# SCZwangxiao/video-ReTaKe

Measured on NVIDIA B200. Metric: 2048-frame DPSelect+PivotKV frames/s, higher is better.
Workload: dtype bf16

## Files before the change

video-retake_b200/csrc/pivot_misc.cu:

```cuda
#include <climits>

#include <stdlib.h>

#include "rtk_common.cuh"

namespace rtk {

struct RopeParams {
    int heads, L, D, n_pos, forward;
    long long stride_h, stride_l, out_stride_h, out_stride_l;
    int heads2;
    const __nv_bfloat16* x2;
    __nv_bfloat16* out2;
    long long stride_h2, stride_l2, out_stride_h2, out_stride_l2;
    int bound[6];
    float inv_scale2;
};

static bool mrope_bounds(int n_pos, const int32_t* sec, int64_t D, int bound[6]) {
    int acc = 0;
    for (int i = 0; i < 6; ++i) {
        acc += n_pos == 3 ? sec[i % 3] : 0;
        bound[i] = acc;
    }
    return n_pos != 3 || acc == D;
}

__device__ __forceinline__ int rope_pos_row(const RopeParams& p, int c) {
    if (p.n_pos == 1) return 0;
    int i = 0;
    while (i < 5 && c >= p.bound[i]) ++i;
    return i % 3;
}

__global__ void __launch_bounds__(256)
pivot_rope_table_kernel(const long long* __restrict__ pos, const float* __restrict__ inv_freq, RopeParams p, float scaling,
                        __nv_bfloat16* __restrict__ cos_t, __nv_bfloat16* __restrict__ sin_t) {
    pdl_enter();
    const int half = p.D >> 1;
    const long long total = (long long)p.L * p.D;
    for (long long i = (long long)blockIdx.x * blockDim.x + threadIdx.x; i < total; i += (long long)gridDim.x * blockDim.x) {
        const int c = (int)(i % p.D);
        const int l = (int)(i / p.D);
        const long long pv = pos[(size_t)rope_pos_row(p, c) * p.L + l];
        const float ang = inv_freq[c < half ? c : c - half] * (float)pv;
        cos_t[i] = __float2bfloat16_rn(cosf(ang) * scaling);
        sin_t[i] = __float2bfloat16_rn(sinf(ang) * scaling);
    }
}

__device__ __forceinline__ void rope_rotate_pair(float xa, float xb, float cosa, float sina, float cosb, float sinb, int forward,
                                                 float inv_scale2, __nv_bfloat16& oa, __nv_bfloat16& ob) {
    const float ta = round_bf16(xa * cosa), ra = round_bf16(-xb * sina);
    const float tb = round_bf16(xb * cosb), rb = round_bf16(xa * sinb);
    float ya, yb;
    if (forward) {
        ya = ta + ra;
        yb = tb + rb;
    } else {
        ya = round_bf16(ta - ra) * inv_scale2;
        yb = round_bf16(tb - rb) * inv_scale2;
    }
    oa = __float2bfloat16_rn(ya);
    ob = __float2bfloat16_rn(yb);
}

__device__ __forceinline__ void rope_table_entry(const RopeParams& p, const float* __restrict__ inv_freq, const long long* pv,
                                                 int c, float scaling, float& co, float& si) {
    const int half = p.D >> 1;
    const float ang = inv_freq[c < half ? c : c - half] * (float)pv[rope_pos_row(p, c)];
    co = __bfloat162float(__float2bfloat16_rn(cosf(ang) * scaling));
    si = __bfloat162float(__float2bfloat16_rn(sinf(ang) * scaling));
}

#ifndef RTK_UNROPE_TOK
#define RTK_UNROPE_TOK 2
#endif
constexpr int kUnropeTok = RTK_UNROPE_TOK;

__device__ __forceinline__ uint32_t sub_bf16x2_rn(uint32_t a, uint32_t b) {
    uint32_t d;
    asm("sub.rn.bf16x2 %0, %1, %2;" : "=r"(d) : "r"(a), "r"(b));
    return d;
}
__device__ __forceinline__ uint32_t add_bf16x2_rn(uint32_t a, uint32_t b) {
    uint32_t d;
    asm("add.rn.bf16x2 %0, %1, %2;" : "=r"(d) : "r"(a), "r"(b));
    return d;
}
__device__ __forceinline__ void unrotate_bf16x2(uint32_t xa, uint32_t xb, uint32_t cs, uint32_t sn, bool scale, float inv_scale2,
                                                uint32_t& oa, uint32_t& ob) {
    const uint32_t ta = mul_bf16x2_rn(xa, cs), ra = mul_bf16x2_rn(xb ^ 0x80008000u, sn);
    const uint32_t tb = mul_bf16x2_rn(xb, cs), rb = mul_bf16x2_rn(xa, sn);
    oa = sub_bf16x2_rn(ta, ra);
    ob = sub_bf16x2_rn(tb, rb);
    if (scale) {
        oa = scale_bf16x2_rn(oa, inv_scale2);
        ob = scale_bf16x2_rn(ob, inv_scale2);
    }
}

__device__ __forceinline__ void unrope_qk_body(const __nv_bfloat16* __restrict__ x, const long long* __restrict__ pos,
                                               const float* __restrict__ inv_freq, float scaling,
                                               __nv_bfloat16* __restrict__ out, const RopeParams& p) {
    __shared__ __align__(16) __nv_bfloat16 s_cos[kUnropeTok][128], s_sin[kUnropeTok][128];
    const int half = p.D >> 1;
    const int vec_per_row = half >> 3;
    const int ntask = (p.heads + p.heads2) * vec_per_row;
    const int tid = threadIdx.x;
    const bool scale = p.inv_scale2 != 1.0f;
    const int v0 = tid % vec_per_row, h0 = tid / vec_per_row;
    const bool second0 = h0 >= p.heads;
    const long long src_h0 = second0 ? (long long)(h0 - p.heads) * p.stride_h2 : (long long)h0 * p.stride_h;
    const long long src_l0 = second0 ? p.stride_l2 : p.stride_l;
    const __nv_bfloat16* src0 = (second0 ? p.x2 : x) + src_h0 + v0 * 8;
    for (int l0 = blockIdx.x * kUnropeTok; l0 < p.L; l0 += gridDim.x * kUnropeTok) {
        const int nl = min(kUnropeTok, p.L - l0);
        uint4 lo4[kUnropeTok], hi4[kUnropeTok];
        if (tid < ntask) {
#pragma unroll
            for (int t = 0; t < kUnropeTok; ++t) {
                if (t < nl) {
                    lo4[t] = *reinterpret_cast<const uint4*>(src0 + (l0 + t) * src_l0);
                    hi4[t] = *reinterpret_cast<const uint4*>(src0 + (l0 + t) * src_l0 + half);
                }
            }
        }
        for (int e = tid; e < nl * half; e += blockDim.x) {
            const int t = e / half, c = e - t * half;
            long long pv[3] = {0, 0, 0};
            for (int r = 0; r < p.n_pos; ++r) pv[r] = pos[(size_t)r * p.L + l0 + t];
            float co, si;
            rope_table_entry(p, inv_freq, pv, c, scaling, co, si);
            s_cos[t][c] = __float2bfloat16_rn(co);
            s_sin[t][c] = __float2bfloat16_rn(si);
        }
        __syncthreads();
#pragma unroll
        for (int t = 0; t < kUnropeTok; ++t) {
            if (t >= nl) break;
            const int l = l0 + t;
            for (int task = tid; task < ntask; task += blockDim.x) {
                const int v = task % vec_per_row, h = task / vec_per_row;
                const int c0 = v * 8;
                const bool second = h >= p.heads;
                const __nv_bfloat16* src = second ? p.x2 + (h - p.heads) * p.stride_h2 + l * p.stride_l2 : x + h * p.stride_h + l * p.stride_l;
                __nv_bfloat16* dst = second ? p.out2 + (h - p.heads) * p.out_stride_h2 + l * p.out_stride_l2
                                            : out + h * p.out_stride_h + l * p.out_stride_l;
                uint4 a4 = lo4[t], b4 = hi4[t];
                if (task != tid) {
                    a4 = *reinterpret_cast<const uint4*>(src + c0);
                    b4 = *reinterpret_cast<const uint4*>(src + c0 + half);
                }
                const uint4 cs = *reinterpret_cast<const uint4*>(&s_cos[t][c0]);
                const uint4 sn = *reinterpret_cast<const uint4*>(&s_sin[t][c0]);
                uint4 ol4, oh4;
                unrotate_bf16x2(a4.x, b4.x, cs.x, sn.x, scale, p.inv_scale2, ol4.x, oh4.x);
                unrotate_bf16x2(a4.y, b4.y, cs.y, sn.y, scale, p.inv_scale2, ol4.y, oh4.y);
                unrotate_bf16x2(a4.z, b4.z, cs.z, sn.z, scale, p.inv_scale2, ol4.z, oh4.z);
                unrotate_bf16x2(a4.w, b4.w, cs.w, sn.w, scale, p.inv_scale2, ol4.w, oh4.w);
                *reinterpret_cast<uint4*>(dst + c0) = ol4;
                *reinterpret_cast<uint4*>(dst + c0 + half) = oh4;
            }
        }
        __syncthreads();
    }
}

struct BatchLayers {
    const __nv_bfloat16* q[kMaxBatchLayers];
    const __nv_bfloat16* k[kMaxBatchLayers];
    const __nv_bfloat16* k_in[kMaxBatchLayers];
    const __nv_bfloat16* v[kMaxBatchLayers];
    __nv_bfloat16* qu[kMaxBatchLayers];
    __nv_bfloat16* ku[kMaxBatchLayers];
    const long long* pos[kMaxBatchLayers];
    const uint8_t* keymask[kMaxBatchLayers];
    __nv_bfloat16* k_out[kMaxBatchLayers];
    __nv_bfloat16* v_out[kMaxBatchLayers];
    long long* pos_out[kMaxBatchLayers];
    int32_t* keep_idx[kMaxBatchLayers];
    const __nv_bfloat16* head_scores[kMaxBatchLayers];
    long long q_stride_h[kMaxBatchLayers], q_stride_l[kMaxBatchLayers];
    long long kin_stride_h[kMaxBatchLayers], kin_stride_l[kMaxBatchLayers];
    long long k_stride_h[kMaxBatchLayers], k_stride_l[kMaxBatchLayers];
    long long v_stride_h[kMaxBatchLayers], v_stride_l[kMaxBatchLayers];
    long long out_stride_h[kMaxBatchLayers], pos_out_stride[kMaxBatchLayers];
};

__global__ void __launch_bounds__(256)
pivot_unrope_qk_batch_kernel(const __grid_constant__ BatchLayers t, const float* __restrict__ inv_freq, float scaling, RopeParams p) {
    pdl_enter();
    const int layer = blockIdx.y;
    p.stride_h = t.q_stride_h[layer]; p.stride_l = t.q_stride_l[layer];
    p.x2 = t.k_in[layer]; p.out2 = t.ku[layer];
    p.stride_h2 = t.kin_stride_h[layer]; p.stride_l2 = t.kin_stride_l[layer];
    unrope_qk_body(t.q[layer], t.pos[layer], inv_freq, scaling, t.qu[layer], p);
}

__global__ void __launch_bounds__(256)
pivot_rope_kernel(const __nv_bfloat16* __restrict__ x, const __nv_bfloat16* __restrict__ cos_t,
                  const __nv_bfloat16* __restrict__ sin_t, __nv_bfloat16* __restrict__ out, RopeParams p) {
    pdl_enter();
    const int half = p.D >> 1;
    const int vec_per_row = half >> 3;
    const long long total = (long long)(p.heads + p.heads2) * p.L * vec_per_row;
    for (long long i = (long long)blockIdx.x * blockDim.x + threadIdx.x; i < total; i += (long long)gridDim.x * blockDim.x) {
        const int v = (int)(i % vec_per_row);
        const long long hl = i / vec_per_row;
        const int l = (int)(hl % p.L);
        const int h = (int)(hl / p.L);
        const int c0 = v * 8;
        const bool second = h >= p.heads;
        const __nv_bfloat16* src = second ? p.x2 + (h - p.heads) * p.stride_h2 + l * p.stride_l2 : x + h * p.stride_h + l * p.stride_l;
        __nv_bfloat16* dst = second ? p.out2 + (h - p.heads) * p.out_stride_h2 + l * p.out_stride_l2
                                    : out + h * p.out_stride_h + l * p.out_stride_l;
        uint4 lo4 = *reinterpret_cast<const uint4*>(src + c0);
        uint4 hi4 = *reinterpret_cast<const uint4*>(src + c0 + half);
        const __nv_bfloat16* xl = reinterpret_cast<const __nv_bfloat16*>(&lo4);
        const __nv_bfloat16* xh = reinterpret_cast<const __nv_bfloat16*>(&hi4);
        uint4 ol4, oh4;
        __nv_bfloat16* ol = reinterpret_cast<__nv_bfloat16*>(&ol4);
        __nv_bfloat16* oh = reinterpret_cast<__nv_bfloat16*>(&oh4);
        const int rowa0 = rope_pos_row(p, c0), rowa1 = rope_pos_row(p, c0 + 7);
        const int rowb0 = rope_pos_row(p, c0 + half), rowb1 = rope_pos_row(p, c0 + half + 7);
        uint4 ca4, sa4, cb4, sb4;
        __nv_bfloat16* cav = reinterpret_cast<__nv_bfloat16*>(&ca4);
        __nv_bfloat16* sav = reinterpret_cast<__nv_bfloat16*>(&sa4);
        __nv_bfloat16* cbv = reinterpret_cast<__nv_bfloat16*>(&cb4);
        __nv_bfloat16* sbv = reinterpret_cast<__nv_bfloat16*>(&sb4);
        if (rowa0 == rowa1 && rowb0 == rowb1) {
            const size_t ia = ((size_t)rowa0 * p.L + l) * p.D + c0, ib = ((size_t)rowb0 * p.L + l) * p.D + c0 + half;
            ca4 = __ldg(reinterpret_cast<const uint4*>(cos_t + ia));
            sa4 = __ldg(reinterpret_cast<const uint4*>(sin_t + ia));
            cb4 = __ldg(reinterpret_cast<const uint4*>(cos_t + ib));
            sb4 = __ldg(reinterpret_cast<const uint4*>(sin_t + ib));
        } else {
#pragma unroll
            for (int e = 0; e < 8; ++e) {
                const int ca = c0 + e, cb = c0 + e + half;
                const size_t ia = ((size_t)rope_pos_row(p, ca) * p.L + l) * p.D + ca;
                const size_t ib = ((size_t)rope_pos_row(p, cb) * p.L + l) * p.D + cb;
                cav[e] = cos_t[ia]; sav[e] = sin_t[ia]; cbv[e] = cos_t[ib]; sbv[e] = sin_t[ib];
            }
        }
#pragma unroll
        for (int e = 0; e < 8; ++e)
            rope_rotate_pair(__bfloat162float(xl[e]), __bfloat162float(xh[e]), __bfloat162float(cav[e]), __bfloat162float(sav[e]),
                             __bfloat162float(cbv[e]), __bfloat162float(sbv[e]), p.forward, p.inv_scale2, ol[e], oh[e]);
        *reinterpret_cast<uint4*>(dst + c0) = ol4;
        *reinterpret_cast<uint4*>(dst + c0 + half) = oh4;
    }
}

bool key_elision_enabled();

struct KeyElide {
    const uint8_t* keymask[kMaxBatchLayers];
    int32_t* slot[kMaxBatchLayers];
    const __nv_bfloat16* k[kMaxBatchLayers];
    long long k_stride_h[kMaxBatchLayers], k_stride_l[kMaxBatchLayers];
    __nv_bfloat16* kc[kMaxBatchLayers];
    int32_t* n_keys;
    int L, KVH, D;
};

__global__ void __launch_bounds__(1024)
pivot_keymask_scan_kernel(const __grid_constant__ KeyElide e) {
    pdl_enter();
    __shared__ int wsum[32];
    const int layer = blockIdx.x, tid = threadIdx.x, lane = tid & 31, warp = tid >> 5;
    const uint8_t* __restrict__ m = e.keymask[layer];
    int32_t* __restrict__ slot = e.slot[layer];
    const int per = (e.L + 1023) / 1024;
    const int beg = min(tid * per, e.L), end = min(beg + per, e.L);
    int cnt = 0;
    for (int i = beg; i < end; ++i) cnt += !(m && m[i]);
    int inc = cnt;
#pragma unroll
    for (int o = 1; o < 32; o <<= 1) {
        const int n = __shfl_up_sync(0xffffffffu, inc, o);
        if (lane >= o) inc += n;
    }
    if (lane == 31) wsum[warp] = inc;
    __syncthreads();
    if (warp == 0) {
        const int w = wsum[lane];
        int winc = w;
#pragma unroll
        for (int o = 1; o < 32; o <<= 1) {
            const int n = __shfl_up_sync(0xffffffffu, winc, o);
            if (lane >= o) winc += n;
        }
        wsum[lane] = winc - w;
        if (lane == 31) e.n_keys[layer] = winc;
    }
    __syncthreads();
    int base = wsum[warp] + inc - cnt;
    for (int i = beg; i < end; ++i) slot[i] = (m && m[i]) ? -1 : base++;
}

__global__ void __launch_bounds__(256)
pivot_keys_compact_kernel(const __grid_constant__ KeyElide e) {
    pdl_enter();
    const int layer = blockIdx.y;
    const int vpr = e.D >> 3;
    const long long total = (long long)e.L * e.KVH * vpr;
    const int32_t* __restrict__ slot = e.slot[layer];
    for (long long i = (long long)blockIdx.x * blockDim.x + threadIdx.x; i < total; i += (long long)gridDim.x * blockDim.x) {
        const int v = (int)(i % vpr);
        const long long lh = i / vpr;
        const int h = (int)(lh % e.KVH);
        const int l = (int)(lh / e.KVH);
        const int sl = slot[l];
        if (sl < 0) continue;
        const uint4 w = __ldg(reinterpret_cast<const uint4*>(e.k[layer] + h * e.k_stride_h[layer] + l * e.k_stride_l[layer] + v * 8));
        *reinterpret_cast<uint4*>(e.kc[layer] + ((size_t)sl * e.KVH + h) * e.D + v * 8) = w;
    }
}

static int key_elide_prepare(KeyElide& ke, int n, ScoreBatch& sb, cudaStream_t st) {
    RTK_LAUNCH_PDL(pivot_keymask_scan_kernel, (unsigned)n, 1024, 0, st, ke);
    const long long total = (long long)ke.L * ke.KVH * (ke.D >> 3);
    long long gx = (total + 255) / 256;
    if (gx > 148 * 8) gx = 148 * 8;
    RTK_LAUNCH_PDL(pivot_keys_compact_kernel, dim3((unsigned)gx, (unsigned)n), 256, 0, st, ke);
    for (int i = 0; i < n; ++i) {
        sb.kc[i] = ke.kc[i];
        sb.slot[i] = ke.slot[i];
    }
    sb.n_keys = ke.n_keys;
    return 0;
}

static size_t key_elide_bytes(int64_t KVH, int64_t L, int64_t D) {
    return (((size_t)KVH * L * D * 2 + 255) & ~(size_t)255) + (((size_t)L * 4 + 255) & ~(size_t)255);
}

constexpr int kSelThreads = 1024;

__device__ void block_select_top(const uint32_t* keys, int L, int keep, int32_t* out_idx, int* sh ,
                                 int low_bit ) {
    const int tid = threadIdx.x, lane = tid & 31, warp = tid >> 5;
    const int per = (L + kSelThreads - 1) / kSelThreads;
    const int beg = min(tid * per, L), end = min(beg + per, L);
    uint32_t prefix = 0;
    for (int bit = 31; bit >= low_bit; --bit) {
        const uint32_t cand = prefix | (1u << bit);
        int cnt = 0;
        for (int i = beg; i < end; ++i) cnt += (keys[i] >= cand);
        cnt = __reduce_add_sync(0xffffffffu, cnt);
        int* buf = sh + 40 + 32 * (bit & 1);
        if (lane == 0) buf[warp] = cnt;
        __syncthreads();
        const int total = __reduce_add_sync(0xffffffffu, buf[lane]);
        if (total >= keep) prefix = cand;
    }
    __syncthreads();
    if (low_bit > 0 && (!(prefix & 0x80000000u) || (prefix >> low_bit) == (0xffffffffu >> low_bit)))
        prefix |= (1u << low_bit) - 1u;
    int gt = 0, eq = 0;
    for (int i = beg; i < end; ++i) { gt += (keys[i] > prefix); eq += (keys[i] == prefix); }
    auto block_excl_scan = [&](int v, int& total) {
        int inc = v;
#pragma unroll
        for (int o = 1; o < 32; o <<= 1) {
            const int n = __shfl_up_sync(0xffffffffu, inc, o);
            if (lane >= o) inc += n;
        }
        __syncthreads();
        if (lane == 31) sh[1 + warp] = inc;
        __syncthreads();
        if (warp == 0) {
            int w = sh[1 + lane], winc = w;
#pragma unroll
            for (int o = 1; o < 32; o <<= 1) {
                const int n = __shfl_up_sync(0xffffffffu, winc, o);
                if (lane >= o) winc += n;
            }
            sh[1 + lane] = winc - w;
            if (lane == 31) sh[33] = winc;
        }
        __syncthreads();
        total = sh[33];
        return sh[1 + warp] + inc - v;
    };
    int gt_total, eq_total;
    const int gt_before = block_excl_scan(gt, gt_total);
    const int eq_before = block_excl_scan(eq, eq_total);
    const int need = keep - gt_total;
    const int eq_taken_before = min(eq_before, need);
    int slot = gt_before + eq_taken_before;
    int eq_seen = eq_before;
    for (int i = beg; i < end; ++i) {
        const uint32_t k = keys[i];
        bool take = k > prefix;
        if (k == prefix) { take = eq_seen < need; ++eq_seen; }
        if (take) out_idx[slot++] = i;
    }
}

__device__ __forceinline__ void pivot_select_body(const __nv_bfloat16* __restrict__ head_scores, int KVH, int L,
                                                  const uint8_t* __restrict__ keymask, int keep, int32_t* __restrict__ keep_idx,
                                                  __nv_bfloat16* __restrict__ score_out, const long long* __restrict__ tpos,
                                                  long long* __restrict__ tmin_out) {
    extern __shared__ __align__(128) uint8_t smem[];
    uint32_t* keys = reinterpret_cast<uint32_t*>(smem);
    int* sh = reinterpret_cast<int*>(smem + (size_t)L * 4);
    const float rcp = 1.0f / (float)KVH;
    for (int i = threadIdx.x; i < L; i += blockDim.x) {
        float v[4] = {0.f, 0.f, 0.f, 0.f};
        for (int j = 0; j < KVH; ++j) v[j & 3] += __bfloat162float(head_scores[(size_t)j * L + i]);
        const __nv_bfloat16 s = __float2bfloat16_rn((((v[0] + v[1]) + v[2]) + v[3]) * rcp);
        if (score_out) score_out[i] = s;
        const float f = (keymask && keymask[i]) ? 1.0f : __bfloat162float(s);
        keys[i] = f32_to_ordered(f);
    }
// ... 302 lines not shown
    if (grid > 148 * 16) grid = 148 * 16;
    RTK_LAUNCH_PDL(pivot_rope_kernel, (unsigned)grid, 256, 0, st, (const __nv_bfloat16*)x, (const __nv_bfloat16*)cos, (const __nv_bfloat16*)sin, (__nv_bfloat16*)out, p);
    return 0;
}

extern "C" int rtk_pivot_rope(const void* x, int64_t heads, int64_t L, int64_t D, int64_t stride_h, int64_t stride_l,
                              const void* cos, const void* sin, int n_pos, const int32_t* mrope_section_host,
                              float inv_scale2, int forward, void* out, int64_t out_stride_h, int64_t out_stride_l,
                              void* stream) {
    RTK_NVTX("rtk_pivot_rope");
    if (!x || !cos || !sin || !out || heads < 1 || L < 1 || D < 16) return RTK_E_BADARG;
    if (D % 16 != 0 || (n_pos != 1 && n_pos != 3)) return RTK_E_UNSUPPORTED;
    if (n_pos == 3 && !mrope_section_host) return RTK_E_BADARG;
    if ((((uintptr_t)x | (uintptr_t)out) & 15u) != 0) return RTK_E_ALIGN;
    if ((stride_h | stride_l | out_stride_h | out_stride_l) % 8 != 0) return RTK_E_ALIGN;
    RopeParams p;
    p.heads = (int)heads; p.L = (int)L; p.D = (int)D; p.n_pos = n_pos; p.forward = forward;
    p.stride_h = stride_h; p.stride_l = stride_l; p.out_stride_h = out_stride_h; p.out_stride_l = out_stride_l;
    p.inv_scale2 = inv_scale2;
    p.heads2 = 0; p.x2 = nullptr; p.out2 = nullptr;
    p.stride_h2 = p.stride_l2 = p.out_stride_h2 = p.out_stride_l2 = 0;
    if (!mrope_bounds(n_pos, mrope_section_host, D, p.bound)) return RTK_E_UNSUPPORTED;
    return rope_launch(x, cos, sin, out, p, (cudaStream_t)stream);
}

extern "C" int rtk_pivot_select(const void* head_scores, int64_t KVH, int64_t L, const uint8_t* keymask, int64_t keep,
                                int32_t* keep_idx, void* score_out, void* stream) {
    RTK_NVTX("rtk_pivot_select");
    if (!head_scores || !keep_idx || KVH < 1 || L < 1 || keep < 1 || keep > L) return RTK_E_BADARG;
    if (L > 16384) return RTK_E_UNSUPPORTED;
    const size_t smem = (size_t)L * 4 + 112 * 4;
    cudaError_t e = cudaFuncSetAttribute(pivot_select_kernel, cudaFuncAttributeMaxDynamicSharedMemorySize, (int)smem);
    if (e != cudaSuccess) return (int)e;
    RTK_LAUNCH_PDL(pivot_select_kernel, 1, kSelThreads, smem, (cudaStream_t)stream, (const __nv_bfloat16*)head_scores, (int)KVH,
                   (int)L, keymask, (int)keep, keep_idx, (__nv_bfloat16*)score_out);
    return 0;
}

extern "C" int rtk_pivot_compact(const void* k, const void* v, int64_t KVH, int64_t L, int64_t D, int64_t stride_h,
                                 int64_t stride_l, const int32_t* keep_idx, int64_t keep, void* k_out, void* v_out,
                                 int64_t out_stride_h, const int64_t* pos, int n_pos, int64_t* pos_out, int reforge,
                                 void* stream) {
    RTK_NVTX("rtk_pivot_compact");
    if ((!k && !v) || !keep_idx || (k && !k_out) || (v && !v_out) || KVH < 1 || L < 1 || D < 8 || keep < 1 || keep > L)
        return RTK_E_BADARG;
    if (pos && (!pos_out || n_pos < 1)) return RTK_E_BADARG;
    if (D % 8 != 0) return RTK_E_UNSUPPORTED;
    if ((((uintptr_t)k | (uintptr_t)v | (uintptr_t)k_out | (uintptr_t)v_out) & 15u) != 0) return RTK_E_ALIGN;
    if ((stride_h | stride_l | out_stride_h) % 8 != 0) return RTK_E_ALIGN;
    CompactParams p;
    p.KVH = (int)KVH; p.L = (int)L; p.D = (int)D; p.keep = (int)keep; p.n_pos = n_pos; p.reforge = reforge;
    p.stride_h = stride_h; p.stride_l = stride_l; p.out_stride_h = out_stride_h;
    p.v_stride_h = stride_h; p.v_stride_l = stride_l;
    p.pos_out_stride = keep;
    p.ratio = (float)((double)keep / (double)L);
    const long long total = KVH * keep * (D / 8);
    long long grid = (total + 255) / 256;
    if (grid > 148 * 8) grid = 148 * 8;
    RTK_LAUNCH_PDL(pivot_compact_kernel, (unsigned)(grid + 1), 256, 0, (cudaStream_t)stream,  (const __nv_bfloat16*)k, (const __nv_bfloat16*)v, keep_idx, (__nv_bfloat16*)k_out, (__nv_bfloat16*)v_out, (const long long*)pos, (long long*)pos_out, p);
    return 0;
}

extern "C" int rtk_pivot_rope_tables(const int64_t* pos, int n_pos, int64_t L, int64_t D, const float* inv_freq,
                                     const int32_t* mrope_section_host, float attention_scaling, void* cos_out,
                                     void* sin_out, void* stream) {
    RTK_NVTX("rtk_pivot_rope_tables");
    if (!pos || !inv_freq || !cos_out || !sin_out || L < 1 || D < 2) return RTK_E_BADARG;
    if (D % 2 != 0 || (n_pos != 1 && n_pos != 3)) return RTK_E_UNSUPPORTED;
    if (n_pos == 3 && !mrope_section_host) return RTK_E_BADARG;
    RopeParams p;
    p.heads = 1; p.L = (int)L; p.D = (int)D; p.n_pos = n_pos; p.forward = 0;
    p.stride_h = p.stride_l = p.out_stride_h = p.out_stride_l = 0;
    p.heads2 = 0; p.x2 = nullptr; p.out2 = nullptr;
    p.stride_h2 = p.stride_l2 = p.out_stride_h2 = p.out_stride_l2 = 0;
    p.inv_scale2 = 1.0f;
    if (!mrope_bounds(n_pos, mrope_section_host, D, p.bound)) return RTK_E_UNSUPPORTED;
    long long grid = (L * D + 255) / 256;
    if (grid > 148 * 8) grid = 148 * 8;
    RTK_LAUNCH_PDL(pivot_rope_table_kernel, (unsigned)grid, 256, 0, (cudaStream_t)stream,  (const long long*)pos, inv_freq, p, attention_scaling, (__nv_bfloat16*)cos_out, (__nv_bfloat16*)sin_out);
    return 0;
}

static size_t align256(size_t x) { return (x + 255) & ~(size_t)255; }

extern "C" size_t rtk_pivot_update_batch_workspace_bytes(int64_t H, int64_t KVH, int64_t L, int64_t D, int64_t n_layers) {
    if (H < 1 || KVH < 1 || L < 1 || D < 1 || n_layers < 1) return 0;
    const size_t n = (size_t)(n_layers < kMaxBatchLayers ? n_layers : kMaxBatchLayers);
    return align256(rtk_pivot_score_workspace_bytes(H * (int64_t)n, L)) +
           n * (align256((size_t)H * L * D * 2) + align256((size_t)KVH * L * D * 2)) + align256(n * sizeof(long long)) + 256 +
           n * key_elide_bytes(KVH, L, D) + 256;
}

extern "C" size_t rtk_pivot_update_workspace_bytes(int64_t H, int64_t KVH, int64_t L, int64_t D) {
    return rtk_pivot_update_batch_workspace_bytes(H, KVH, L, D, 1);
}

#ifndef RTK_UNROT_TOKEN_MAJOR
#define RTK_UNROT_TOKEN_MAJOR 1
#endif

static int pivot_update_group(const rtk_pivot_update_args* a, int n, char* ws, cudaStream_t st) {
    const rtk_pivot_update_args& a0 = a[0];
    const int64_t H = a0.H, KVH = a0.KVH, L = a0.L, D = a0.D;
    const bool reforge = a0.reforge != 0;
    const int64_t uq_sh = RTK_UNROT_TOKEN_MAJOR ? D : L * D, uq_sl = RTK_UNROT_TOKEN_MAJOR ? H * D : D;
    const int64_t uk_sh = RTK_UNROT_TOKEN_MAJOR ? D : L * D, uk_sl = RTK_UNROT_TOKEN_MAJOR ? KVH * D : D;
    void* score_ws = ws;                ws += align256(rtk_pivot_score_workspace_bytes(H * n, L));
    char* qu0 = ws;                     ws += (size_t)n * align256((size_t)H * L * D * 2);
    char* ku0 = ws;                     ws += (size_t)n * align256((size_t)KVH * L * D * 2);
    long long* tmin = (long long*)ws;   ws += align256((size_t)n * sizeof(long long)) + 256;
    char* kc0 = ws;                     ws += (size_t)n * align256((size_t)KVH * L * D * 2);
    char* slot0 = ws;                   ws += (size_t)n * align256((size_t)L * 4);
    int32_t* nkeys_ws = (int32_t*)ws;

    BatchLayers t = {};
    ScoreBatch sb = {};
    sb.n = n; sb.H = H; sb.KVH = KVH; sb.L = L; sb.D = D;
    for (int i = 0; i < kMaxBatchLayers; ++i) {
        const rtk_pivot_update_args& x = a[i < n ? i : 0];
        char* qu = qu0 + (size_t)(i < n ? i : 0) * align256((size_t)H * L * D * 2);
        char* ku = ku0 + (size_t)(i < n ? i : 0) * align256((size_t)KVH * L * D * 2);
        t.q[i] = (const __nv_bfloat16*)x.q;       t.q_stride_h[i] = x.q_stride_h;     t.q_stride_l[i] = x.q_stride_l;
        t.k_in[i] = (const __nv_bfloat16*)x.k;    t.kin_stride_h[i] = x.k_stride_h;   t.kin_stride_l[i] = x.k_stride_l;
        t.qu[i] = (__nv_bfloat16*)qu;             t.ku[i] = (__nv_bfloat16*)ku;
        t.k[i] = reforge ? (const __nv_bfloat16*)ku : (const __nv_bfloat16*)x.k;
        t.k_stride_h[i] = reforge ? uk_sh : x.k_stride_h;
        t.k_stride_l[i] = reforge ? uk_sl : x.k_stride_l;
        t.v[i] = (const __nv_bfloat16*)x.v;       t.v_stride_h[i] = x.v_stride_h;     t.v_stride_l[i] = x.v_stride_l;
        t.pos[i] = (const long long*)x.pos;       t.keymask[i] = x.keymask;
        t.k_out[i] = (__nv_bfloat16*)x.k_out;     t.v_out[i] = (__nv_bfloat16*)x.v_out;
        t.out_stride_h[i] = x.out_stride_h;
        t.pos_out[i] = (long long*)x.pos_out;     t.pos_out_stride[i] = x.pos_out_stride > 0 ? x.pos_out_stride : x.keep;
        t.keep_idx[i] = x.keep_idx;               t.head_scores[i] = (const __nv_bfloat16*)x.head_scores;
        if (i < n) {
            sb.q[i] = reforge ? (const void*)qu : x.q;
            sb.k[i] = reforge ? (const void*)ku : x.k;
            sb.q_stride_h[i] = reforge ? uq_sh : x.q_stride_h;   sb.q_stride_l[i] = reforge ? uq_sl : x.q_stride_l;
            sb.k_stride_h[i] = reforge ? uk_sh : x.k_stride_h;   sb.k_stride_l[i] = reforge ? uk_sl : x.k_stride_l;
            sb.head_scores[i] = x.head_scores;
        }
    }
    RopeParams rp = {};
    rp.heads = (int)H; rp.L = (int)L; rp.D = (int)D; rp.n_pos = a0.n_pos; rp.forward = 0;
    rp.out_stride_h = uq_sh; rp.out_stride_l = uq_sl;
    rp.heads2 = (int)KVH; rp.out_stride_h2 = uk_sh; rp.out_stride_l2 = uk_sl;
    rp.inv_scale2 = a0.inv_scale2;
    mrope_bounds(a0.n_pos, a0.mrope_section, D, rp.bound);
    const bool xchg = a0.xchg_world > 1;
    const int64_t score_rows = a0.score_rows > 0 ? a0.score_rows : KVH;
    if (reforge && !a0.skip_score) {
        if (a0.inv_freq) {
            RTK_LAUNCH_PDL(pivot_unrope_qk_batch_kernel, dim3((unsigned)((L + kUnropeTok - 1) / kUnropeTok), (unsigned)n), 256, 0, st, t, a0.inv_freq,
                           a0.attention_scaling, rp);
        } else {
            rp.stride_h = a0.q_stride_h; rp.stride_l = a0.q_stride_l;
            rp.x2 = t.k_in[0]; rp.out2 = t.ku[0]; rp.stride_h2 = a0.k_stride_h; rp.stride_l2 = a0.k_stride_l;
            const int rc = rope_launch(a0.q, a0.cos, a0.sin, t.qu[0], rp, st);
            if (rc) return rc;
        }
    }
    if (!a0.skip_score) {
        bool any_mask = false;
        for (int i = 0; i < n; ++i) any_mask = any_mask || a[i].keymask != nullptr;
        if (any_mask && key_elision_enabled()) {
            KeyElide ke = {};
            ke.L = (int)L; ke.KVH = (int)KVH; ke.D = (int)D; ke.n_keys = nkeys_ws;
            for (int i = 0; i < kMaxBatchLayers; ++i) {
                const int j = i < n ? i : 0;
                ke.keymask[i] = a[j].keymask;
                ke.slot[i] = (int32_t*)(slot0 + (size_t)j * align256((size_t)L * 4));
                ke.k[i] = t.k[j]; ke.k_stride_h[i] = t.k_stride_h[j]; ke.k_stride_l[i] = t.k_stride_l[j];
                ke.kc[i] = (__nv_bfloat16*)(kc0 + (size_t)j * align256((size_t)KVH * L * D * 2));
            }
            int rc = key_elide_prepare(ke, n, sb, st);
            if (rc) return rc;
        }
        if (a0.ev_score_begin) cudaEventRecord((cudaEvent_t)a0.ev_score_begin, st);
        int rc = pivot_score_batch(sb, score_ws, rtk_pivot_score_workspace_bytes(H * n, L), st);
        if (rc) return rc;
        if (a0.ev_score_end) cudaEventRecord((cudaEvent_t)a0.ev_score_end, st);
    }
    if (a0.skip_select) {
        if (xchg) {
            XchgPutBatch xp = {};
            xp.n = (long long)KVH * L; xp.world = a0.xchg_world; xp.rank = a0.xchg_rank;
            for (int i = 0; i < n; ++i) {
                xp.src[i] = (const __nv_bfloat16*)a[i].head_scores;
                for (int r = 0; r < a0.xchg_world; ++r)
                    xp.dst[i][r] = (__nv_bfloat16*)a[i].xchg_scores[r] + (size_t)a0.xchg_rank * KVH * L;
            }
            RTK_LAUNCH_PDL(pivot_xchg_put_batch_kernel, (unsigned)n, 1024, 0, st, xp);
            XchgFlags xf = {};
            xf.world = a0.xchg_world; xf.rank = a0.xchg_rank; xf.epoch = a0.xchg_epoch;
            for (int r = 0; r < a0.xchg_world; ++r) xf.flags[r] = a0.xchg_flags[r];
            RTK_LAUNCH_PDL(pivot_xchg_flag_kernel, 1, 32, 0, st, xf);
        }
        return 0;
    }
    {
        const size_t smem = (size_t)L * 4 + 112 * 4;
        cudaError_t e = cudaFuncSetAttribute(pivot_select_batch_kernel, cudaFuncAttributeMaxDynamicSharedMemorySize, (int)smem);
        if (e != cudaSuccess) return (int)e;
        RTK_LAUNCH_PDL(pivot_select_batch_kernel, (unsigned)n, kSelThreads, smem, st, t, (int)score_rows, (int)L, (int)a0.keep,
                       reforge ? 1 : 0, tmin, (const uint32_t*)(xchg ? a0.xchg_flags[a0.xchg_rank] : nullptr),
                       xchg ? a0.xchg_world : 0, a0.xchg_epoch, xchg_timeout_ns());
    }
    {
        CompactParams p = {};
        p.KVH = (int)KVH; p.L = (int)L; p.D = (int)D; p.keep = (int)a0.keep; p.n_pos = a0.pos ? a0.n_pos : 0; p.reforge = a0.reforge;
        p.ratio = (float)((double)a0.keep / (double)L);
        RopeParams rq = {};
        rq.D = (int)D; rq.n_pos = a0.n_pos; rq.L = (int)a0.keep;
        for (int i = 0; i < 6; ++i) rq.bound[i] = rp.bound[i];
        RTK_LAUNCH_PDL(pivot_compact_rope_batch_kernel, dim3((unsigned)a0.keep, (unsigned)n), 128, 0, st, t, (const long long*)tmin,
                       a0.inv_freq, a0.attention_scaling, p, rq, (reforge && a0.inv_freq) ? 1 : 0);
    }
    return 0;
}

static int update_check(const rtk_pivot_update_args* layers, int64_t n, const void* workspace, size_t workspace_bytes) {
    if (!layers || n < 1 || !workspace) return RTK_E_BADARG;
    const rtk_pivot_update_args& a0 = layers[0];
    const bool scores = !a0.skip_score, selects = !a0.skip_select, xchg = a0.xchg_world > 1;
    if (!scores && !selects) return RTK_E_BADARG;
    if (a0.H < 1 || a0.KVH < 1 || a0.L < 1 || (selects && (a0.keep < 1 || a0.keep > a0.L))) return RTK_E_BADARG;
    if (a0.L > 16384 || a0.D % 16 != 0 || a0.D > 256) return RTK_E_UNSUPPORTED;
    if (scores && ((a0.D != 64 && a0.D != 128) || a0.H % a0.KVH != 0 || a0.H > 256)) return RTK_E_UNSUPPORTED;
    if (xchg) {
        if (n > kMaxBatchLayers) return RTK_E_UNSUPPORTED;
        if (a0.xchg_world > 8 || a0.xchg_rank < 0 || a0.xchg_rank >= a0.xchg_world || (scores && selects)) return RTK_E_BADARG;
    }
    if (a0.reforge && !a0.inv_freq && n > 1) return RTK_E_UNSUPPORTED;
    int bound[6];
    if (a0.reforge && (scores || a0.inv_freq) && !mrope_bounds(a0.n_pos, a0.mrope_section, a0.D, bound)) return RTK_E_UNSUPPORTED;
    if (((uintptr_t)workspace & 255u) != 0) return RTK_E_ALIGN;
    if (workspace_bytes < rtk_pivot_update_batch_workspace_bytes(a0.H, a0.KVH, a0.L, a0.D, n)) return RTK_E_WORKSPACE;
    for (int64_t i = 0; i < n; ++i) {
        const rtk_pivot_update_args& x = layers[i];
        if (!x.q || !x.k || !x.v || !x.k_out || !x.v_out || !x.keep_idx || !x.head_scores) return RTK_E_BADARG;
        if (x.H != a0.H || x.KVH != a0.KVH || x.L != a0.L || x.D != a0.D || x.keep != a0.keep || x.reforge != a0.reforge ||
            x.n_pos != a0.n_pos || x.inv_freq != a0.inv_freq || x.attention_scaling != a0.attention_scaling ||
            x.inv_scale2 != a0.inv_scale2 || x.skip_select != a0.skip_select || x.skip_score != a0.skip_score ||
            x.score_rows != a0.score_rows || x.xchg_world != a0.xchg_world || x.xchg_rank != a0.xchg_rank ||
            x.xchg_epoch != a0.xchg_epoch || (x.pos == nullptr) != (a0.pos == nullptr))
            return RTK_E_UNSUPPORTED;
        for (int j = 0; j < 3; ++j)
            if (x.mrope_section[j] != a0.mrope_section[j]) return RTK_E_UNSUPPORTED;
        if (x.reforge && (!x.pos || !x.pos_out || (!x.inv_freq && (!x.cos || !x.sin)))) return RTK_E_BADARG;
        if (xchg) {
            for (int r = 0; r < a0.xchg_world; ++r)
                if (!x.xchg_scores[r] || !a0.xchg_flags[r]) return RTK_E_BADARG;
            const char* own = (const char*)x.xchg_scores[a0.xchg_rank];
            if (a0.skip_score && (const char*)x.head_scores != own) return RTK_E_BADARG;
            if (a0.skip_select && (const char*)x.head_scores != own + (size_t)a0.xchg_rank * a0.KVH * a0.L * 2) return RTK_E_BADARG;
        }
        if (x.pos && (selects || x.reforge) && (!x.pos_out || x.n_pos < 1 || x.n_pos > 3)) return RTK_E_BADARG;
        uintptr_t ptrs = 0;
        int64_t strides = 0;
        if (scores) {
            ptrs |= (uintptr_t)x.q;
            strides |= x.q_stride_h | x.q_stride_l;
        }
        if (scores || !x.reforge) {
            ptrs |= (uintptr_t)x.k;
            strides |= x.k_stride_h | x.k_stride_l;
        }
        if (selects) {
            ptrs |= (uintptr_t)x.v | (uintptr_t)x.k_out | (uintptr_t)x.v_out;
            strides |= x.v_stride_h | x.v_stride_l | x.out_stride_h;
        }
        if ((ptrs & 15u) != 0 || strides % 8 != 0) return RTK_E_ALIGN;
    }
    return 0;
}

extern "C" int rtk_pivot_update(const rtk_pivot_update_args* a, void* stream) {
    RTK_NVTX("rtk_pivot_update");
    if (!a) return RTK_E_BADARG;
    const int rc = update_check(a, 1, a->workspace, a->workspace_bytes);
    if (rc) return rc;
    return pivot_update_group(a, 1, (char*)a->workspace, (cudaStream_t)stream);
}

extern "C" int rtk_pivot_update_batch(const rtk_pivot_update_args* layers, int64_t n_layers, void* workspace,
                                      size_t workspace_bytes, void* stream) {
    RTK_NVTX("rtk_pivot_update_batch");
    int rc = update_check(layers, n_layers, workspace, workspace_bytes);
    if (rc) return rc;
    for (int64_t i = 0; i < n_layers; i += kMaxBatchLayers) {
        const int n = (int)((n_layers - i) < kMaxBatchLayers ? (n_layers - i) : kMaxBatchLayers);
        rc = pivot_update_group(layers + i, n, (char*)workspace, (cudaStream_t)stream);
        if (rc) return rc;
    }
    return 0;
}

extern "C" int rtk_kv_block_copy(int n_jobs, const void* const* src, void* const* dst, const int64_t* heads, const int64_t* rows,
                                 const int64_t* src_stride_h, const int64_t* src_stride_l, const int64_t* dst_stride_h,
                                 const int64_t* dst_stride_l, int64_t D, void* stream) {
    RTK_NVTX("rtk_kv_block_copy");
    if (n_jobs < 1 || n_jobs > 4 || !src || !dst || !heads || !rows || D < 8) return RTK_E_BADARG;
    if (D % 8 != 0) return RTK_E_UNSUPPORTED;
    CopyJobs j;
    j.n = n_jobs;
    j.D = (int)D;
    long long acc = 0;
    for (int k = 0; k < n_jobs; ++k) {
        if (!src[k] || !dst[k] || heads[k] < 1 || rows[k] < 0) return RTK_E_BADARG;
        if ((((uintptr_t)src[k] | (uintptr_t)dst[k]) & 15u) != 0) return RTK_E_ALIGN;
        if ((src_stride_h[k] | src_stride_l[k] | dst_stride_h[k] | dst_stride_l[k]) % 8 != 0) return RTK_E_ALIGN;
        j.src[k] = (const __nv_bfloat16*)src[k];
        j.dst[k] = (__nv_bfloat16*)dst[k];
        j.heads[k] = (int)heads[k];
        j.rows[k] = (int)rows[k];
        j.src_stride_h[k] = src_stride_h[k]; j.src_stride_l[k] = src_stride_l[k];
        j.dst_stride_h[k] = dst_stride_h[k]; j.dst_stride_l[k] = dst_stride_l[k];
        acc += heads[k] * rows[k] * (D / 8);
// ... 10 lines not shown
```

Measured before the change: 3613.

## Precompute deduplicated unrope cos/sin tables and fuse key compaction into unrope

Adds a table kernel that reduces each position row to its min/max. When the values span fewer than L entries, it builds cos/sin tables indexed by position value, so each distinct position is computed once instead of once per token per block. The per-token unrope kernel then reads cos/sin from these global tables instead of computing them in shared memory with a __syncthreads. When key elision is active, the unrope kernel also writes the unroped keys straight into the compacted key buffer, which replaces the separate keys-compact kernel. This costs more workspace and one extra launch, and tokens whose 8-element vector straddles mRoPE sections fall back to gathering scalar table entries.

```diff
diff --git a/video-retake_b200/csrc/pivot_misc.cu b/video-retake_b200/csrc/pivot_misc.cu
--- a/video-retake_b200/csrc/pivot_misc.cu
+++ b/video-retake_b200/csrc/pivot_misc.cu
@@ -77,6 +77,7 @@
 #define RTK_UNROPE_TOK 2
 #endif
 constexpr int kUnropeTok = RTK_UNROPE_TOK;
+constexpr int kUnropeTableCtas = 16;
 
 __device__ __forceinline__ uint32_t sub_bf16x2_rn(uint32_t a, uint32_t b) {
     uint32_t d;
@@ -100,72 +101,22 @@
     }
 }
 
-__device__ __forceinline__ void unrope_qk_body(const __nv_bfloat16* __restrict__ x, const long long* __restrict__ pos,
-                                               const float* __restrict__ inv_freq, float scaling,
-                                               __nv_bfloat16* __restrict__ out, const RopeParams& p) {
-    __shared__ __align__(16) __nv_bfloat16 s_cos[kUnropeTok][128], s_sin[kUnropeTok][128];
-    const int half = p.D >> 1;
-    const int vec_per_row = half >> 3;
-    const int ntask = (p.heads + p.heads2) * vec_per_row;
-    const int tid = threadIdx.x;
-    const bool scale = p.inv_scale2 != 1.0f;
-    const int v0 = tid % vec_per_row, h0 = tid / vec_per_row;
-    const bool second0 = h0 >= p.heads;
-    const long long src_h0 = second0 ? (long long)(h0 - p.heads) * p.stride_h2 : (long long)h0 * p.stride_h;
-    const long long src_l0 = second0 ? p.stride_l2 : p.stride_l;
-    const __nv_bfloat16* src0 = (second0 ? p.x2 : x) + src_h0 + v0 * 8;
-    for (int l0 = blockIdx.x * kUnropeTok; l0 < p.L; l0 += gridDim.x * kUnropeTok) {
-        const int nl = min(kUnropeTok, p.L - l0);
-        uint4 lo4[kUnropeTok], hi4[kUnropeTok];
-        if (tid < ntask) {
-#pragma unroll
-            for (int t = 0; t < kUnropeTok; ++t) {
-                if (t < nl) {
-                    lo4[t] = *reinterpret_cast<const uint4*>(src0 + (l0 + t) * src_l0);
-                    hi4[t] = *reinterpret_cast<const uint4*>(src0 + (l0 + t) * src_l0 + half);
-                }
-            }
-        }
-        for (int e = tid; e < nl * half; e += blockDim.x) {
-            const int t = e / half, c = e - t * half;
-            long long pv[3] = {0, 0, 0};
-            for (int r = 0; r < p.n_pos; ++r) pv[r] = pos[(size_t)r * p.L + l0 + t];
-            float co, si;
-            rope_table_entry(p, inv_freq, pv, c, scaling, co, si);
-            s_cos[t][c] = __float2bfloat16_rn(co);
-            s_sin[t][c] = __float2bfloat16_rn(si);
-        }
-        __syncthreads();
-#pragma unroll
-        for (int t = 0; t < kUnropeTok; ++t) {
-            if (t >= nl) break;
-            const int l = l0 + t;
-            for (int task = tid; task < ntask; task += blockDim.x) {
-                const int v = task % vec_per_row, h = task / vec_per_row;
-                const int c0 = v * 8;
-                const bool second = h >= p.heads;
-                const __nv_bfloat16* src = second ? p.x2 + (h - p.heads) * p.stride_h2 + l * p.stride_l2 : x + h * p.stride_h + l * p.stride_l;
-                __nv_bfloat16* dst = second ? p.out2 + (h - p.heads) * p.out_stride_h2 + l * p.out_stride_l2
-                                            : out + h * p.out_stride_h + l * p.out_stride_l;
-                uint4 a4 = lo4[t], b4 = hi4[t];
-                if (task != tid) {
-                    a4 = *reinterpret_cast<const uint4*>(src + c0);
-                    b4 = *reinterpret_cast<const uint4*>(src + c0 + half);
-                }
-                const uint4 cs = *reinterpret_cast<const uint4*>(&s_cos[t][c0]);
-                const uint4 sn = *reinterpret_cast<const uint4*>(&s_sin[t][c0]);
-                uint4 ol4, oh4;
-                unrotate_bf16x2(a4.x, b4.x, cs.x, sn.x, scale, p.inv_scale2, ol4.x, oh4.x);
-                unrotate_bf16x2(a4.y, b4.y, cs.y, sn.y, scale, p.inv_scale2, ol4.y, oh4.y);
-                unrotate_bf16x2(a4.z, b4.z, cs.z, sn.z, scale, p.inv_scale2, ol4.z, oh4.z);
-                unrotate_bf16x2(a4.w, b4.w, cs.w, sn.w, scale, p.inv_scale2, ol4.w, oh4.w);
-                *reinterpret_cast<uint4*>(dst + c0) = ol4;
-                *reinterpret_cast<uint4*>(dst + c0 + half) = oh4;
-            }
-        }
-        __syncthreads();
-    }
-}
+struct UnropeTables {
+    __nv_bfloat16* cos;
+    __nv_bfloat16* sin;
+    long long* base;
+    const int32_t* slot;
+    __nv_bfloat16* kc;
+    long long slot_stride, kc_stride;
+};
+
+__device__ __forceinline__ size_t unrope_entry(const UnropeTables& u, int layer, int r, int L, int half,
+                                               const long long* __restrict__ pos, int l) {
+    const long long base = u.base[layer * 3 + r];
+    const long long e = base == LLONG_MIN ? (long long)l : pos[(size_t)r * L + l] - base;
+    return (((size_t)layer * 3 + r) * L + (size_t)e) * half;
+}
+
 
 struct BatchLayers {
     const __nv_bfloat16* q[kMaxBatchLayers];
@@ -189,13 +140,112 @@
 };
 
 __global__ void __launch_bounds__(256)
-pivot_unrope_qk_batch_kernel(const __grid_constant__ BatchLayers t, const float* __restrict__ inv_freq, float scaling, RopeParams p) {
+pivot_unrope_table_kernel(const __grid_constant__ BatchLayers t, const float* __restrict__ inv_freq, float scaling, RopeParams p,
+                          UnropeTables u) {
+    pdl_enter();
+    __shared__ long long s_mn[8], s_mx[8];
+    const int r = blockIdx.y, layer = blockIdx.z, tid = threadIdx.x, lane = tid & 31, warp = tid >> 5;
+    const long long* __restrict__ row = t.pos[layer] + (size_t)r * p.L;
+    long long mn = LLONG_MAX, mx = LLONG_MIN;
+#pragma unroll 4
+    for (int l = tid; l < p.L; l += blockDim.x) {
+        const long long v = row[l];
+        mn = min(mn, v);
+        mx = max(mx, v);
+    }
+#pragma unroll
+    for (int o = 16; o > 0; o >>= 1) {
+        mn = min(mn, __shfl_xor_sync(0xffffffffu, mn, o));
+        mx = max(mx, __shfl_xor_sync(0xffffffffu, mx, o));
+    }
+    if (lane == 0) { s_mn[warp] = mn; s_mx[warp] = mx; }
+    __syncthreads();
+    for (int w = 0; w < (int)(blockDim.x >> 5); ++w) { mn = min(mn, s_mn[w]); mx = max(mx, s_mx[w]); }
+    const bool by_value = mn != LLONG_MIN && (unsigned long long)mx - (unsigned long long)mn < (unsigned long long)p.L;
+    if (blockIdx.x == 0 && tid == 0) u.base[layer * 3 + r] = by_value ? mn : LLONG_MIN;
+    const int half = p.D >> 1;
+    const int c_lo = (p.n_pos == 1 || r == 0) ? 0 : p.bound[r - 1], c_hi = p.n_pos == 1 ? half : p.bound[r];
+    const int nc = c_hi - c_lo;
+    const long long total = (by_value ? mx - mn + 1 : (long long)p.L) * nc;
+    const size_t off = ((size_t)layer * 3 + r) * p.L * half;
+    for (long long i = (long long)blockIdx.x * blockDim.x + tid; i < total; i += (long long)gridDim.x * blockDim.x) {
+        const int e = (int)(i / nc), c = c_lo + (int)(i - (long long)e * nc);
+        long long pv[3] = {0, 0, 0};
+        pv[r] = by_value ? mn + e : row[e];
+        float co, si;
+        rope_table_entry(p, inv_freq, pv, c, scaling, co, si);
+        u.cos[off + (size_t)e * half + c] = __float2bfloat16_rn(co);
+        u.sin[off + (size_t)e * half + c] = __float2bfloat16_rn(si);
+    }
+}
+
+__global__ void __launch_bounds__(256)
+pivot_unrope_qk_batch_kernel(const __grid_constant__ BatchLayers t, RopeParams p, UnropeTables u) {
     pdl_enter();
     const int layer = blockIdx.y;
-    p.stride_h = t.q_stride_h[layer]; p.stride_l = t.q_stride_l[layer];
-    p.x2 = t.k_in[layer]; p.out2 = t.ku[layer];
-    p.stride_h2 = t.kin_stride_h[layer]; p.stride_l2 = t.kin_stride_l[layer];
-    unrope_qk_body(t.q[layer], t.pos[layer], inv_freq, scaling, t.qu[layer], p);
+    const int half = p.D >> 1, vpr = half >> 3;
+    const int ntask = (p.heads + p.heads2) * vpr;
+    const bool scale = p.inv_scale2 != 1.0f;
+    const long long* __restrict__ pos = t.pos[layer];
+    const int32_t* __restrict__ slot = u.slot ? u.slot + layer * u.slot_stride : nullptr;
+    for (int l0 = blockIdx.x * kUnropeTok; l0 < p.L; l0 += gridDim.x * kUnropeTok) {
+        const int nl = min(kUnropeTok, p.L - l0);
+        for (int task = threadIdx.x; task < ntask; task += blockDim.x) {
+            const int v = task % vpr, h = task / vpr, c0 = v * 8;
+            const bool second = h >= p.heads;
+            const int hh = second ? h - p.heads : h;
+            const __nv_bfloat16* src = second ? t.k_in[layer] + hh * t.kin_stride_h[layer] : t.q[layer] + hh * t.q_stride_h[layer];
+            const long long src_l = second ? t.kin_stride_l[layer] : t.q_stride_l[layer];
+            __nv_bfloat16* dst = second ? t.ku[layer] + hh * p.out_stride_h2 : t.qu[layer] + hh * p.out_stride_h;
+            const long long dst_l = second ? p.out_stride_l2 : p.out_stride_l;
+            const int r0 = rope_pos_row(p, c0);
+            const bool one_row = r0 == rope_pos_row(p, c0 + 7);
+            uint4 a4[kUnropeTok], b4[kUnropeTok], cs[kUnropeTok], sn[kUnropeTok];
+            int sl[kUnropeTok];
+#pragma unroll
+            for (int j = 0; j < kUnropeTok; ++j) {
+                if (j >= nl) break;
+                const int l = l0 + j;
+                a4[j] = *reinterpret_cast<const uint4*>(src + l * src_l + c0);
+                b4[j] = *reinterpret_cast<const uint4*>(src + l * src_l + c0 + half);
+                sl[j] = (second && slot) ? slot[l] : -1;
+                if (one_row) {
+                    const size_t o = unrope_entry(u, layer, r0, p.L, half, pos, l) + c0;
+                    cs[j] = *reinterpret_cast<const uint4*>(u.cos + o);
+                    sn[j] = *reinterpret_cast<const uint4*>(u.sin + o);
+                } else {
+                    unsigned long long cw[2] = {0, 0}, sw[2] = {0, 0};
+#pragma unroll 1
+                    for (int e = 0; e < 8; ++e) {
+                        const size_t o = unrope_entry(u, layer, rope_pos_row(p, c0 + e), p.L, half, pos, l) + c0 + e;
+                        const int sh = 16 * (e & 3);
+                        const unsigned long long cb = __bfloat16_as_ushort(u.cos[o]), sb = __bfloat16_as_ushort(u.sin[o]);
+                        if (e < 4) { cw[0] |= cb << sh; sw[0] |= sb << sh; }
+                        else       { cw[1] |= cb << sh; sw[1] |= sb << sh; }
+                    }
+                    cs[j] = make_uint4((uint32_t)cw[0], (uint32_t)(cw[0] >> 32), (uint32_t)cw[1], (uint32_t)(cw[1] >> 32));
+                    sn[j] = make_uint4((uint32_t)sw[0], (uint32_t)(sw[0] >> 32), (uint32_t)sw[1], (uint32_t)(sw[1] >> 32));
+                }
+            }
+#pragma unroll
+            for (int j = 0; j < kUnropeTok; ++j) {
+                if (j >= nl) break;
+                const int l = l0 + j;
+                uint4 ol4, oh4;
+                unrotate_bf16x2(a4[j].x, b4[j].x, cs[j].x, sn[j].x, scale, p.inv_scale2, ol4.x, oh4.x);
+                unrotate_bf16x2(a4[j].y, b4[j].y, cs[j].y, sn[j].y, scale, p.inv_scale2, ol4.y, oh4.y);
+                unrotate_bf16x2(a4[j].z, b4[j].z, cs[j].z, sn[j].z, scale, p.inv_scale2, ol4.z, oh4.z);
+                unrotate_bf16x2(a4[j].w, b4[j].w, cs[j].w, sn[j].w, scale, p.inv_scale2, ol4.w, oh4.w);
+                *reinterpret_cast<uint4*>(dst + l * dst_l + c0) = ol4;
+                *reinterpret_cast<uint4*>(dst + l * dst_l + c0 + half) = oh4;
+                if (sl[j] >= 0) {
+                    __nv_bfloat16* kc = u.kc + layer * u.kc_stride + ((size_t)sl[j] * p.heads2 + hh) * p.D;
+                    *reinterpret_cast<uint4*>(kc + c0) = ol4;
+                    *reinterpret_cast<uint4*>(kc + c0 + half) = oh4;
+                }
+            }
+        }
+    }
 }
 
 __global__ void __launch_bounds__(256)
@@ -319,20 +369,6 @@
     }
 }
 
-static int key_elide_prepare(KeyElide& ke, int n, ScoreBatch& sb, cudaStream_t st) {
-    RTK_LAUNCH_PDL(pivot_keymask_scan_kernel, (unsigned)n, 1024, 0, st, ke);
-    const long long total = (long long)ke.L * ke.KVH * (ke.D >> 3);
-    long long gx = (total + 255) / 256;
-    if (gx > 148 * 8) gx = 148 * 8;
-    RTK_LAUNCH_PDL(pivot_keys_compact_kernel, dim3((unsigned)gx, (unsigned)n), 256, 0, st, ke);
-    for (int i = 0; i < n; ++i) {
-        sb.kc[i] = ke.kc[i];
-        sb.slot[i] = ke.slot[i];
-    }
-    sb.n_keys = ke.n_keys;
-    return 0;
-}
-
 static size_t key_elide_bytes(int64_t KVH, int64_t L, int64_t D) {
     return (((size_t)KVH * L * D * 2 + 255) & ~(size_t)255) + (((size_t)L * 4 + 255) & ~(size_t)255);
 }
@@ -801,13 +837,14 @@
 }
 
 static size_t align256(size_t x) { return (x + 255) & ~(size_t)255; }
+static size_t unrope_plane_bytes(size_t n, int64_t L, int64_t D) { return align256(n * 3 * (size_t)L * (size_t)(D / 2) * 2); }
 
 extern "C" size_t rtk_pivot_update_batch_workspace_bytes(int64_t H, int64_t KVH, int64_t L, int64_t D, int64_t n_layers) {
     if (H < 1 || KVH < 1 || L < 1 || D < 1 || n_layers < 1) return 0;
     const size_t n = (size_t)(n_layers < kMaxBatchLayers ? n_layers : kMaxBatchLayers);
     return align256(rtk_pivot_score_workspace_bytes(H * (int64_t)n, L)) +
            n * (align256((size_t)H * L * D * 2) + align256((size_t)KVH * L * D * 2)) + align256(n * sizeof(long long)) + 256 +
-           n * key_elide_bytes(KVH, L, D) + 256;
+           n * key_elide_bytes(KVH, L, D) + 256 + 2 * unrope_plane_bytes(n, L, D) + align256(n * 3 * sizeof(long long));
 }
 
 extern "C" size_t rtk_pivot_update_workspace_bytes(int64_t H, int64_t KVH, int64_t L, int64_t D) {
@@ -830,7 +867,11 @@
     long long* tmin = (long long*)ws;   ws += align256((size_t)n * sizeof(long long)) + 256;
     char* kc0 = ws;                     ws += (size_t)n * align256((size_t)KVH * L * D * 2);
     char* slot0 = ws;                   ws += (size_t)n * align256((size_t)L * 4);
-    int32_t* nkeys_ws = (int32_t*)ws;
+    int32_t* nkeys_ws = (int32_t*)ws;   ws += 256;
+    UnropeTables ut = {};
+    ut.cos = (__nv_bfloat16*)ws;        ws += unrope_plane_bytes(n, L, D);
+    ut.sin = (__nv_bfloat16*)ws;        ws += unrope_plane_bytes(n, L, D);
+    ut.base = (long long*)ws;
 
     BatchLayers t = {};
     ScoreBatch sb = {};
@@ -867,33 +908,49 @@
     mrope_bounds(a0.n_pos, a0.mrope_section, D, rp.bound);
     const bool xchg = a0.xchg_world > 1;
     const int64_t score_rows = a0.score_rows > 0 ? a0.score_rows : KVH;
-    if (reforge && !a0.skip_score) {
-        if (a0.inv_freq) {
-            RTK_LAUNCH_PDL(pivot_unrope_qk_batch_kernel, dim3((unsigned)((L + kUnropeTok - 1) / kUnropeTok), (unsigned)n), 256, 0, st, t, a0.inv_freq,
-                           a0.attention_scaling, rp);
-        } else {
-            rp.stride_h = a0.q_stride_h; rp.stride_l = a0.q_stride_l;
-            rp.x2 = t.k_in[0]; rp.out2 = t.ku[0]; rp.stride_h2 = a0.k_stride_h; rp.stride_l2 = a0.k_stride_l;
-            const int rc = rope_launch(a0.q, a0.cos, a0.sin, t.qu[0], rp, st);
-            if (rc) return rc;
-        }
+    bool elide = false;
+    if (!a0.skip_score && key_elision_enabled())
+        for (int i = 0; i < n; ++i) elide = elide || a[i].keymask != nullptr;
+    KeyElide ke = {};
+    if (elide) {
+        ke.L = (int)L; ke.KVH = (int)KVH; ke.D = (int)D; ke.n_keys = nkeys_ws;
+        for (int i = 0; i < kMaxBatchLayers; ++i) {
+            const int j = i < n ? i : 0;
+            ke.keymask[i] = a[j].keymask;
+            ke.slot[i] = (int32_t*)(slot0 + (size_t)j * align256((size_t)L * 4));
+            ke.k[i] = t.k[j]; ke.k_stride_h[i] = t.k_stride_h[j]; ke.k_stride_l[i] = t.k_stride_l[j];
+            ke.kc[i] = (__nv_bfloat16*)(kc0 + (size_t)j * align256((size_t)KVH * L * D * 2));
+        }
+        RTK_LAUNCH_PDL(pivot_keymask_scan_kernel, (unsigned)n, 1024, 0, st, ke);
+        for (int i = 0; i < n; ++i) {
+            sb.kc[i] = ke.kc[i];
+            sb.slot[i] = ke.slot[i];
+        }
+        sb.n_keys = ke.n_keys;
+    }
+    const bool unrope_fast = reforge && !a0.skip_score && a0.inv_freq;
+    if (unrope_fast) {
+        if (elide) {
+            ut.slot = ke.slot[0]; ut.slot_stride = (long long)(align256((size_t)L * 4) / 4);
+            ut.kc = ke.kc[0];     ut.kc_stride = (long long)(align256((size_t)KVH * L * D * 2) / 2);
+        }
+        RTK_LAUNCH_PDL(pivot_unrope_table_kernel, dim3(kUnropeTableCtas, (unsigned)a0.n_pos, (unsigned)n), 256, 0, st, t, a0.inv_freq,
+                       a0.attention_scaling, rp, ut);
+        RTK_LAUNCH_PDL(pivot_unrope_qk_batch_kernel, dim3((unsigned)((L + kUnropeTok - 1) / kUnropeTok), (unsigned)n), 256, 0, st, t,
+                       rp, ut);
+    } else if (reforge && !a0.skip_score) {
+        rp.stride_h = a0.q_stride_h; rp.stride_l = a0.q_stride_l;
+        rp.x2 = t.k_in[0]; rp.out2 = t.ku[0]; rp.stride_h2 = a0.k_stride_h; rp.stride_l2 = a0.k_stride_l;
+        const int rc = rope_launch(a0.q, a0.cos, a0.sin, t.qu[0], rp, st);
+        if (rc) return rc;
+    }
+    if (elide && !unrope_fast) {
+        const long long total = L * KVH * (D >> 3);
+        long long gx = (total + 255) / 256;
+        if (gx > 148 * 8) gx = 148 * 8;
+        RTK_LAUNCH_PDL(pivot_keys_compact_kernel, dim3((unsigned)gx, (unsigned)n), 256, 0, st, ke);
     }
     if (!a0.skip_score) {
-        bool any_mask = false;
-        for (int i = 0; i < n; ++i) any_mask = any_mask || a[i].keymask != nullptr;
-        if (any_mask && key_elision_enabled()) {
-            KeyElide ke = {};
-            ke.L = (int)L; ke.KVH = (int)KVH; ke.D = (int)D; ke.n_keys = nkeys_ws;
-            for (int i = 0; i < kMaxBatchLayers; ++i) {
-                const int j = i < n ? i : 0;
-                ke.keymask[i] = a[j].keymask;
-                ke.slot[i] = (int32_t*)(slot0 + (size_t)j * align256((size_t)L * 4));
-                ke.k[i] = t.k[j]; ke.k_stride_h[i] = t.k_stride_h[j]; ke.k_stride_l[i] = t.k_stride_l[j];
-                ke.kc[i] = (__nv_bfloat16*)(kc0 + (size_t)j * align256((size_t)KVH * L * D * 2));
-            }
-            int rc = key_elide_prepare(ke, n, sb, st);
-            if (rc) return rc;
-        }
         if (a0.ev_score_begin) cudaEventRecord((cudaEvent_t)a0.ev_score_begin, st);
         int rc = pivot_score_batch(sb, score_ws, rtk_pivot_score_workspace_bytes(H * n, L), st);
         if (rc) return rc;
@@ -951,7 +1008,9 @@
     }
     if (a0.reforge && !a0.inv_freq && n > 1) return RTK_E_UNSUPPORTED;
     int bound[6];
-    if (a0.reforge && (scores || a0.inv_freq) && !mrope_bounds(a0.n_pos, a0.mrope_section, a0.D, bound)) return RTK_E_UNSUPPORTED;
+    if (a0.reforge && (scores || a0.inv_freq) &&
+        ((a0.n_pos != 1 && a0.n_pos != 3) || !mrope_bounds(a0.n_pos, a0.mrope_section, a0.D, bound)))
+        return RTK_E_UNSUPPORTED;
     if (((uintptr_t)workspace & 255u) != 0) return RTK_E_ALIGN;
     if (workspace_bytes < rtk_pivot_update_batch_workspace_bytes(a0.H, a0.KVH, a0.L, a0.D, n)) return RTK_E_WORKSPACE;
     for (int64_t i = 0; i < n; ++i) {
```

Result: no change. 3633 (median of 6 runs) (+0.6%).
